# VITA-Group/Open-L2O

Measured on AMD Instinct MI355X. Metric: unroll-steps/sec (batch x params x T), L2O-DM on Quadratic d=128, higher is better.
Workload: dtype f32

## Files before the change

### open_l2o_amd/csrc/l2o_unroll.hip

```cpp
#include "l2o_host.h"
#include "l2o_step.h"
#include "l2o_problem_fg.h"
#include "l2o_unroll.h"
#include "l2o_unroll_pair.h"
#include "l2o_unroll_lds.h"
#include "l2o_unroll_cu.h"
#include "l2o_unroll_cu8.h"
#include "l2o_ilp_kernels.h"

__global__ void k_combine_halves(const float* __restrict__ fx_half, float* __restrict__ fx_part, int nb, int nparts,
                                 float inv_bg, float* __restrict__ fx, unsigned long long* __restrict__ xbuf, long xwords,
                                 PairWs* ws, int b0, int B_local);
__global__ void k_coresident_probe(unsigned* ctr, unsigned* min_seen);

static int check_problem(const l2o_problem* p) {
  if (!p) return fail(L2O_ERR_ARG, "problem is NULL");
  if (p->B_local <= 0 || p->B_global < p->B_local || p->D <= 0)
    return fail(L2O_ERR_ARG, "bad problem sizes B_local=%d B_global=%d D=%d", p->B_local, p->B_global, p->D);
  switch (p->kind) {
    case L2O_PROB_SIMPLE: return L2O_OK;
    case L2O_PROB_QUADRATIC:
    case L2O_PROB_LASSO:
      if (!p->W || !p->y || p->M <= 0) return fail(L2O_ERR_ARG, "problem needs W, y and M > 0");
      if (p->kind == L2O_PROB_QUADRATIC && p->M != p->D) return fail(L2O_ERR_ARG, "quadratic needs M == D");
      return L2O_OK;
    case L2O_PROB_RASTRIGIN:
    case L2O_PROB_SQUARE_COS:
      if (!p->W || !p->y || !p->C || p->M != p->D)
        return fail(L2O_ERR_ARG, "rastrigin / square_cos need W, y, C and M == D");
      return L2O_OK;
    default: return fail(L2O_ERR_UNSUPPORTED, "problem kind %d has no HIP kernel", p->kind);
  }
}

struct UnrollGeom { int CH, nw; size_t lds; };
static bool unroll_geom(const l2o_problem* p, UnrollGeom* g) {
  const int D = p->D, M = p->M;
  g->nw = tiles_per_problem(D);
  if (g->nw > 8 || M > 16 * g->nw) return false;
  const int need = g->nw;
  g->CH = need <= 1 ? 1 : (need <= 2 ? 2 : (need <= 4 ? 4 : 8));
  const int SQ = 16 * g->CH, S = SQ + 16;
  g->lds = sizeof(float) * (2 * (size_t)SQ * S + 3 * (size_t)SQ + 8);
  return g->lds <= 160 * 1024;
}

static int pair_chunk(const l2o_problem* p, const UnrollGeom& g, hipStream_t s) {
  if (!opt(L2O_OPT_PAIR) || g.CH < 2) return 0;
  const int cap = coresident_cus(s) / 2;
  if (p->B_local <= cap) return p->B_local;
  if (cap < 8) return 0;
  const int n = (p->B_local + cap - 1) / cap;
  const int chunk = (((p->B_local + n - 1) / n) + 7) & ~7;
  return chunk <= cap ? chunk : (cap & ~7);
}
struct PairLayout { size_t xbuf_off, xbuf_bytes, fxh_off, total; int npg; size_t lds; };
static PairLayout pair_layout(const l2o_problem* p, const UnrollGeom& g, int T) {
  PairLayout L;
  const int SQ = 16 * g.CH;
  L.npg = SQ;
  L.xbuf_off = sizeof(PairWs);
  L.xbuf_bytes = (size_t)p->B_local * 2 * 2 * L.npg * sizeof(unsigned long long);
  L.fxh_off = L.xbuf_off + L.xbuf_bytes;
  L.total = L.fxh_off + sizeof(float) * (size_t)(T + 1) * g.CH * p->B_local;
  L.lds = 0;
  return L;
}

template <int PRE, int KIND>
static int launch_unroll_ch(const UnrollArgs& a, const UnrollGeom& g, hipStream_t s, const l2o_problem* prob,
                            void* workspace, float* fx, bool* fx_done) {
  const bool hist = a.hist_st != nullptr;
  int chunk = workspace ? pair_chunk(prob, g, s) : 0;
  {
    const int one_lds = (int)opt(L2O_OPT_ONE_LDS);
#ifdef L2O_LDS_ABL_ANYNW
    const bool shape_ok = g.nw >= 1 && a.pp.M <= 16 * g.nw;
#else
    const bool shape_ok = g.CH == 8 && g.nw >= 5;
#endif
    const bool plain = !(opt(L2O_OPT_EXACT_GATES) && !hist);
    if ((one_lds == 2 || (one_lds == 1 && (chunk == 0 || a.pp.B_local > chunk))) && shape_ok && plain) {
      UnrollArgs al = a;
      al.ticks = workspace ? &reinterpret_cast<PairWs*>(workspace)->ticks : nullptr;
      void (*fl)(UnrollArgs) = hist ? k_unroll_lds<PRE, KIND, true> : k_unroll_lds<PRE, KIND, false>;
      const size_t lds = sizeof(float) * ((size_t)LstmCoreLds<PRE>::kFragWords + 2 * 128 + 8);
      const int rc = launch(fl, dim3(a.pp.B_local), dim3(64 * g.nw), lds, s, al);
      if (rc) return rc;
      note_form(L2O_FORM_UNROLL_LDS);
      note_variant(0, hist, false, false, 0, 0);
      return L2O_OK;
    }
  }
  if (chunk > 0) {
    const PairLayout L = pair_layout(prob, g, a.T);
    UnrollPairArgs pa;
    pa.u = a;
    pa.ws = reinterpret_cast<PairWs*>(workspace);
    pa.xbuf = reinterpret_cast<unsigned long long*>(static_cast<char*>(workspace) + L.xbuf_off);
    pa.fx_half = reinterpret_cast<float*>(static_cast<char*>(workspace) + L.fxh_off);
    pa.use_salt = a.T + 1 < 0xffff ? 1u : 0u;
    pa.plain_stores = opt(L2O_OPT_PAIR_PLAIN_STORES) ? 1u : 0u;
    pa.b0 = 0;
    pa.nb = a.pp.B_local;
    const int B = a.pp.B_local;
    const bool one_launch = chunk >= B;
    const bool exact = opt(L2O_OPT_EXACT_GATES) != 0 && !hist;
    bool fast_launched = false;
    {
      void (*fn)(UnrollPairArgs) = nullptr;
      const size_t dyn_lds = L.lds;
      const int SQ = 16 * g.CH;
      const bool fast = opt(L2O_OPT_PAIR_FAST_LOAD) != 0 && a.pp.M == SQ && a.pp.D == SQ;
      pa.fast_load = fast ? 1u : 0u;
      fast_launched = fast;
#define L2O_PAIR_FN(C)                                                                                       \
  (fast ? (hist ? k_unroll_pair<PRE, KIND, C, true, false, true>                                             \
                : (exact ? k_unroll_pair<PRE, KIND, C, false, true, true> : k_unroll_pair<PRE, KIND, C, false, false, true>)) \
        : (hist ? k_unroll_pair<PRE, KIND, C, true> : (exact ? k_unroll_pair<PRE, KIND, C, false, true> : k_unroll_pair<PRE, KIND, C, false>)))
      switch (g.CH) {
        case 2: fn = L2O_PAIR_FN(2); break;
        case 4: fn = L2O_PAIR_FN(4); break;
        default: fn = L2O_PAIR_FN(8); break;
      }
#undef L2O_PAIR_FN
      for (int b0 = 0; b0 < B; b0 += chunk) {
        pa.b0 = b0;
        pa.nb = B - b0 < chunk ? B - b0 : chunk;
        hipLaunchKernelGGL(fn, dim3((pa.nb + 7) / 8 * 16), dim3(64 * (g.CH / 2)), dyn_lds, s, pa);
        HIP_TRY(hipGetLastError());
        hipLaunchKernelGGL(k_combine_halves, dim3(a.T + 1), dim3(256), 0, s, pa.fx_half, a.fx_part, pa.nb, g.CH,
                           a.pp.inv_bg, one_launch ? fx : nullptr, pa.xbuf, (long)pa.nb * 2 * 2 * L.npg, pa.ws, b0, B);
        HIP_TRY(hipGetLastError());
      }
    }
    note_form(L2O_FORM_UNROLL_PAIR, (B + chunk - 1) / chunk);
    note_variant(g.CH, hist, exact, fast_launched, 0, 0);
    if (fx_done) *fx_done = fx != nullptr && one_launch;
    return L2O_OK;
  }
  void (*fn)(UnrollArgs) = nullptr;
  const bool exact1 = opt(L2O_OPT_EXACT_GATES) != 0 && !hist;
  switch (g.CH) {
    case 1: fn = hist ? k_unroll<PRE, KIND, 1, true> : (exact1 ? k_unroll<PRE, KIND, 1, false, true> : k_unroll<PRE, KIND, 1, false>); break;
    case 2: fn = hist ? k_unroll<PRE, KIND, 2, true> : (exact1 ? k_unroll<PRE, KIND, 2, false, true> : k_unroll<PRE, KIND, 2, false>); break;
    case 4: fn = hist ? k_unroll<PRE, KIND, 4, true> : (exact1 ? k_unroll<PRE, KIND, 4, false, true> : k_unroll<PRE, KIND, 4, false>); break;
    default: fn = hist ? k_unroll<PRE, KIND, 8, true> : k_unroll<PRE, KIND, 8, false>; break;
  }
  const int rc = launch(fn, dim3(a.pp.B_local), dim3(64 * g.nw), g.lds, s, a);
  if (rc) return rc;
  note_form(L2O_FORM_UNROLL);
  note_variant(g.CH, hist, exact1 && g.CH <= 4, false, 0, 0);
  return L2O_OK;
}

template <int PRE>
static int launch_unroll_kind(const UnrollArgs& a, const UnrollGeom& g, int kind, hipStream_t s,
                              const l2o_problem* prob, void* workspace, float* fx, bool* fx_done) {
  switch (kind) {
    case L2O_PROB_QUADRATIC: return launch_unroll_ch<PRE, L2O_PROB_QUADRATIC>(a, g, s, prob, workspace, fx, fx_done);
    case L2O_PROB_LASSO: return launch_unroll_ch<PRE, L2O_PROB_LASSO>(a, g, s, prob, workspace, fx, fx_done);
    case L2O_PROB_RASTRIGIN: return launch_unroll_ch<PRE, L2O_PROB_RASTRIGIN>(a, g, s, prob, workspace, fx, fx_done);
    case L2O_PROB_SQUARE_COS: return launch_unroll_ch<PRE, L2O_PROB_SQUARE_COS>(a, g, s, prob, workspace, fx, fx_done);
    default: return fail(L2O_ERR_UNSUPPORTED, "no fused kernel for problem kind %d", kind);
  }
}

static bool unroll_cu_eligible(const l2o_problem* p) {
  if (!opt(L2O_OPT_UNROLL_CU)) return false;
  if (p->D < 4 || p->D > 512 || (p->D & 3) || p->M <= 0) return false;
  return unroll_cu_layout(p->D).lds + sizeof(float) * bx::kBiasWords <= 160 * 1024;
}
template <int PRE, int KR>
static int launch_unroll_cu8(const UnrollArgs& a, hipStream_t s) {
  const UnrollCu8Layout L = unroll_cu8_layout(a.pp.D, PRE, KR);
  const bool hist = a.hist_st != nullptr;
  void (*fn)(UnrollArgs) = a.pp.D <= 256 ? (hist ? k_unroll_cu8<PRE, 1, KR, true> : k_unroll_cu8<PRE, 1, KR, false>)
                                         : (hist ? k_unroll_cu8<PRE, 2, KR, true> : k_unroll_cu8<PRE, 2, KR, false>);
  note_form(L2O_FORM_UNROLL_CU8);
  note_variant(0, hist, false, false, KR, a.pp.D <= 256 ? 1 : 2);
  return launch(fn, dim3(a.pp.B_local), dim3(kCu8Threads), L.lds, s, a);
}
template <int PRE>
static int launch_unroll_cu(const UnrollArgs& a_in, hipStream_t s) {
  const int form = (int)opt(L2O_OPT_UNROLL_CU);
  const bool hist0 = a_in.hist_st != nullptr;
  auto fits = [&](int kr) { return unroll_cu8_layout(a_in.pp.D, PRE, kr).lds + sizeof(float) * bx::kBiasWords <= 160 * 1024; };
  int KR = 0;
  if (form == 1) {
    KR = hist0 ? 2 : (PRE == L2O_PRE_FC_ELU ? 4 : 3);
    if (hist0 && !fits(2) && PRE != L2O_PRE_FC_ELU) KR = 3;
  } else if (form >= 3 && form <= 5) KR = 7 - form;
  if (KR && fits(KR))
    return KR == 4 ? launch_unroll_cu8<PRE, 4>(a_in, s) : (KR == 3 ? launch_unroll_cu8<PRE, 3>(a_in, s) : launch_unroll_cu8<PRE, 2>(a_in, s));
  const UnrollCuLayout L = unroll_cu_layout(a_in.pp.D);
  const UnrollArgs& a = a_in;
  const bool hist = a.hist_st != nullptr;
  void (*fn)(UnrollArgs) = a.pp.D <= 256 ? (hist ? k_unroll_cu<PRE, 1, true> : k_unroll_cu<PRE, 1, false>)
                                         : (hist ? k_unroll_cu<PRE, 2, true> : k_unroll_cu<PRE, 2, false>);
  note_form(L2O_FORM_UNROLL_CU);
  note_variant(0, hist, false, false, 0, a.pp.D <= 256 ? 1 : 2);
  return launch(fn, dim3(a.pp.B_local), dim3(kCuThreads), L.lds, s, a);
}

extern "C" {

static int launch_problem_fg(const ProbParams& pp, const float* x, float* f_part, float* g, void* stream) {
  const size_t lds = sizeof(float) * ((size_t)((pp.D + 3) & ~3) + ((pp.M + 3) & ~3) + 4 * kFgThreads + kFgWaves);
  if (lds > 160 * 1024) return fail(L2O_ERR_UNSUPPORTED, "problem too large for k_problem_fg (D=%d M=%d)", pp.D, pp.M);
  const bool vec = pp.kind != L2O_PROB_SIMPLE && (pp.D & 3) == 0 && ((uintptr_t)pp.W & 15) == 0;
  if (vec && pp.D >= 64 && pp.D <= 2048 && ((uintptr_t)x & 15) == 0 && (!pp.x_scale || ((uintptr_t)pp.x_scale & 15) == 0) &&
      !pp.w_shared && !opt(L2O_OPT_FG_TWO_PASS)) {
    const size_t lds1 = sizeof(float) * ((size_t)kFgWaves * pp.D + kFgWaves);
    void (*f1)(ProbParams, const float*, float*, float*) =
        pp.D <= 256 ? k_problem_fg1<1> : pp.D <= 512 ? k_problem_fg1<2> : pp.D <= 1024 ? k_problem_fg1<4> : k_problem_fg1<8>;
// ... 250 lines not shown
```

### open_l2o_amd/csrc/l2o_unroll_pair.h

```cpp
#pragma once
#include "l2o_lstm_bx3.h"
#include "l2o_params.h"

struct PairWs {
  unsigned status;
  unsigned seq;
  unsigned fault;
  unsigned pad0;
  long long ticks;
  long long ticks_total;
  unsigned pad[8];
  long long phases[16];
};
static_assert(sizeof(PairWs) == 64 + 128, "workspace header layout (include/l2o_abi.h)");

struct UnrollPairArgs {
  UnrollArgs u;
  PairWs* ws;
  unsigned long long* xbuf;
  float* fx_half;
  unsigned use_salt;
  unsigned plain_stores;
  int b0, nb;
  unsigned fast_load;
};

__device__ __forceinline__ unsigned long long pack_granule(float v, unsigned tag) {
  return ((unsigned long long)tag << 32) | (unsigned long long)__float_as_uint(v);
}

template <int N>
__device__ __forceinline__ void lds_read_f4(float4 (&v)[N], const float* p) {
  const unsigned addr = (unsigned)(size_t)(__attribute__((address_space(3))) const char*)p;
  static_assert(N == 1 || N == 2 || N == 4 || N == 8, "");
  if constexpr (N == 1)
    asm volatile("ds_read_b128 %0, %1\n\ts_waitcnt lgkmcnt(0)" : "=&v"(v[0]) : "v"(addr) : "memory");
  if constexpr (N == 2)
    asm volatile("ds_read_b128 %0, %2\n\tds_read_b128 %1, %2 offset:64\n\ts_waitcnt lgkmcnt(0)"
                 : "=&v"(v[0]), "=&v"(v[1]) : "v"(addr) : "memory");
  if constexpr (N == 4)
    asm volatile("ds_read_b128 %0, %4\n\tds_read_b128 %1, %4 offset:64\n\tds_read_b128 %2, %4 offset:128\n\t"
                 "ds_read_b128 %3, %4 offset:192\n\ts_waitcnt lgkmcnt(0)"
                 : "=&v"(v[0]), "=&v"(v[1]), "=&v"(v[2]), "=&v"(v[3]) : "v"(addr) : "memory");
  if constexpr (N == 8)
    asm volatile("ds_read_b128 %0, %8\n\tds_read_b128 %1, %8 offset:64\n\tds_read_b128 %2, %8 offset:128\n\t"
                 "ds_read_b128 %3, %8 offset:192\n\tds_read_b128 %4, %8 offset:256\n\tds_read_b128 %5, %8 offset:320\n\t"
                 "ds_read_b128 %6, %8 offset:384\n\tds_read_b128 %7, %8 offset:448\n\ts_waitcnt lgkmcnt(0)"
                 : "=&v"(v[0]), "=&v"(v[1]), "=&v"(v[2]), "=&v"(v[3]), "=&v"(v[4]), "=&v"(v[5]), "=&v"(v[6]), "=&v"(v[7])
                 : "v"(addr) : "memory");
}

template <int N>
__device__ __forceinline__ void lds_load_f4(l2o::f32x4 (&v)[N], const float* p) {
  const auto* q = reinterpret_cast<const __attribute__((address_space(3))) l2o::f32x4*>(
      (const __attribute__((address_space(3))) float*)p);
#pragma unroll
  for (int m = 0; m < N; ++m) v[m] = q[4 * m];
}
__device__ __forceinline__ void dot4v(const float4 a, const l2o::f32x4 b, float4& acc) {
  acc.x = __builtin_fmaf(a.x, b[0], acc.x);
  acc.y = __builtin_fmaf(a.y, b[1], acc.y);
  acc.z = __builtin_fmaf(a.z, b[2], acc.z);
  acc.w = __builtin_fmaf(a.w, b[3], acc.w);
}

#ifndef L2O_GEMV_PK
#define L2O_GEMV_PK 1
#endif
#ifndef L2O_GEMV_PK_G
#define L2O_GEMV_PK_G L2O_GEMV_PK
#endif
struct Acc4pk { l2o::bx::f32x2 lo, hi; };
__device__ __forceinline__ void dot4pk(const l2o::f32x4 a, const l2o::f32x4 b, Acc4pk& acc) {
  acc.lo = __builtin_elementwise_fma(__builtin_shufflevector(a, a, 0, 1), __builtin_shufflevector(b, b, 0, 1), acc.lo);
  acc.hi = __builtin_elementwise_fma(__builtin_shufflevector(a, a, 2, 3), __builtin_shufflevector(b, b, 2, 3), acc.hi);
}
__device__ __forceinline__ float hsum4pk(const Acc4pk& a) { return (a.lo.x + a.lo.y) + (a.hi.x + a.hi.y); }
__device__ __forceinline__ l2o::f32x4 as_quad(const float4 v) { return l2o::f32x4{v.x, v.y, v.z, v.w}; }
__device__ __forceinline__ void dot4q(const l2o::f32x4 a, const l2o::f32x4 b, float4& acc) {
  acc.x = __builtin_fmaf(a[0], b[0], acc.x);
  acc.y = __builtin_fmaf(a[1], b[1], acc.y);
  acc.z = __builtin_fmaf(a[2], b[2], acc.z);
  acc.w = __builtin_fmaf(a[3], b[3], acc.w);
}

#ifndef L2O_PAIR_LDS_BARRIERS
#define L2O_PAIR_LDS_BARRIERS 0
#endif
#ifdef L2O_PROFILE_PHASES
#define L2O_LAUNCH_MARK(i)                                                                  \
  do {                                                                                      \
    __builtin_amdgcn_sched_barrier(0);                                                      \
    launch_marks[i] = (unsigned)(__builtin_readcyclecounter() - kernel_t0);                 \
    __builtin_amdgcn_sched_barrier(0);                                                      \
  } while (0)
#define L2O_LAUNCH_MARK_LANDED(i)                                                           \
  do {                                                                                      \
    __builtin_amdgcn_sched_barrier(0);                                                      \
    asm volatile("s_waitcnt vmcnt(0) lgkmcnt(0)" ::: "memory");                             \
    L2O_LAUNCH_MARK(i);                                                                     \
  } while (0)
#else
#define L2O_LAUNCH_MARK(i) do {} while (0)
#define L2O_LAUNCH_MARK_LANDED(i) do {} while (0)
#endif

template <int PRE, int KIND, int CH, bool HIST, bool EXACT>
__device__ __forceinline__ void unroll_pair_body_gather(const UnrollPairArgs& pa) {
  const long long kernel_t0 = __builtin_readcyclecounter();
#ifdef L2O_PROFILE_PHASES
  unsigned launch_marks[8] = {0, 0, 0, 0, 0, 0, 0, 0};
#endif
  constexpr int SQ = 16 * CH;
  constexpr int NWH = CH / 2;
  constexpr int NC = 16 * NWH;
  __shared__ __attribute__((aligned(16))) float xs[NC];
  __shared__ __attribute__((aligned(16))) float rs[SQ];
  const UnrollArgs& a = pa.u;
  const ProbParams& pp = a.pp;
  const int D = pp.D, M = pp.M;
  const int tid = threadIdx.x, lane = tid & 63, wv = tid >> 6;
  const int c = lane & 15, q = lane >> 4;
  const int bid = blockIdx.x;
  const unsigned salt = pa.use_salt ? ((pa.ws->seq + 1u) & 0x7fffu) << 16 : 0u;
#ifdef L2O_PROFILE_PHASES
  asm volatile("" ::"s"(salt));
#endif
  L2O_LAUNCH_MARK(0);
  const int half = (bid >> 3) & 1;
  const int bl = ((bid >> 4) << 3) | (bid & 7);
  if (bl >= pa.nb) return;
  const int b = pa.b0 + bl;
  const int tile_in_prob = half * NWH + wv;
  const int gq = q, gr = c;

  const float* Wb = pp.W + (pp.w_shared ? (size_t)0 : (size_t)b * M * D);
  const int col0 = half * NC;
  float4 wr[2][NWH], wt[CH];
#pragma unroll
  for (int p = 0; p < 2; ++p) {
    const int row = (2 * wv + p) * kTile + gr;
#pragma unroll
    for (int m = 0; m < NWH; ++m) {
      float e[4];
#pragma unroll
      for (int k = 0; k < 4; ++k) {
        const int col = col0 + 16 * m + 4 * gq + k;
        e[k] = (row < M && col < D) ? Wb[(size_t)row * D + col] : 0.0f;
      }
      wr[p][m] = make_float4(e[0], e[1], e[2], e[3]);
    }
  }
  {
    const int col = col0 + wv * kTile + gr;
#pragma unroll
    for (int m = 0; m < CH; ++m) {
      float e[4];
#pragma unroll
      for (int k = 0; k < 4; ++k) {
        const int row = 16 * m + 4 * gq + k;
        e[k] = (row < M && col < D) ? Wb[(size_t)row * D + col] : 0.0f;
      }
      wt[m] = make_float4(e[0], e[1], e[2], e[3]);
    }
  }
  constexpr bool kPk = L2O_GEMV_PK != 0;
  l2o::f32x4 wrq[2][NWH], wtq[CH];
#pragma unroll
  for (int m = 0; m < NWH; ++m) { wrq[0][m] = as_quad(wr[0][m]); wrq[1][m] = as_quad(wr[1][m]); }
#pragma unroll
  for (int m = 0; m < CH; ++m) wtq[m] = as_quad(wt[m]);
  const int myrow = (2 * wv + (gq & 1)) * kTile + gr;
  const float myy = (gq < 2 && myrow < M) ? pp.y[(size_t)b * M + myrow] : 0.0f;
  const bool row_counted = gq < 2 && (half == 0 ? (myrow < NC) : (myrow >= NC));

  using Core = LstmCorePair<PRE, !EXACT, false>;
  Core core;
  core.load(a.np.wpack, lane);
  core.pin();
  __shared__ __attribute__((aligned(16))) float bias_s[Core::kBiasFloats];
  core.stage_bias(bias_s, a.np.wpack, tid, blockDim.x, q);
  L2O_LAUNCH_MARK(1);
  const int j = tile_in_prob * kTile + c;
  const bool live = j < D;
  const size_t idx = (size_t)b * D + j;
  const int tpp = (D + kTile - 1) / kTile;
  const bool tile_real = tile_in_prob < tpp;
  TileState s;
  float* st_tile = a.st + ((size_t)b * tpp + (tile_real ? tile_in_prob : 0)) * kStateFloatsPerTile;
  if (tile_real && !a.zero_state) load_tile_state(s, st_tile, lane);
  else {
#pragma unroll
    for (int t = 0; t < kNT; ++t) s.h1[t] = s.c1[t] = s.h2[t] = s.c2[t] = 0.0f;
  }
  float xv = live ? (a.x_in ? a.x_in : a.x)[idx] : 0.0f;
  const float sc = (live && pp.x_scale) ? pp.x_scale[idx] : 1.0f;
  float cj = 0.0f;
  constexpr bool kCos = KIND == L2O_PROB_RASTRIGIN || KIND == L2O_PROB_SQUARE_COS;
  if (kCos) cj = live ? pp.C[idx] : 0.0f;
  float mv = 0.0f, vv = 0.0f;
  if (PRE == L2O_PRE_FC_ELU && !a.zero_state) { mv = live ? a.m[idx] : 0.0f; vv = live ? a.v[idx] : 0.0f; }
  float p1h = a.p1_hi, p1l = a.p1_lo, p2h = a.p2_hi, p2l = a.p2_lo;
  constexpr bool kSq = KIND == L2O_PROB_QUADRATIC || KIND == L2O_PROB_SQUARE_COS;
  const float coef = kSq ? 1.0f : 0.5f;
  const float cg = (KIND == L2O_PROB_QUADRATIC ? 2.0f : 1.0f) * pp.inv_bg;
  const float kTwoPi = pp.twopi;
  const float* xsq = xs + 4 * gq;
  const float* rsq = rs + 4 * gq;
  unsigned long long* mine = pa.xbuf + ((size_t)bl * 2 + half) * 2 * SQ;
  const unsigned long long* theirs = pa.xbuf + ((size_t)bl * 2 + (half ^ 1)) * 2 * SQ;
  bool dead = false;
  if (pa.ws->fault != 0) {
    dead = true;
    if (tid == 0) atomicExch(&pa.ws->status, 1u);
  }
  L2O_LAUNCH_MARK_LANDED(2);
  __shared__ __attribute__((aligned(16))) int same_xcd_s4[4];
  int& same_xcd_s = same_xcd_s4[0];
  if (tid == 0) {
    unsigned my_xcc;
    asm volatile("s_getreg_b32 %0, hwreg(HW_REG_XCC_ID)" : "=s"(my_xcc));
    my_xcc &= 0xfu;
    const unsigned kHsTag = 0x80000000u | salt | 0xffffu;
    __hip_atomic_store(mine + SQ, ((unsigned long long)kHsTag << 32) | my_xcc, __ATOMIC_RELAXED, __HIP_MEMORY_SCOPE_AGENT);
    unsigned long long g = 0;
    int spins = 0;
    bool ok = true;
#pragma nounroll
    for (;;) {
      g = __hip_atomic_load(theirs + SQ, __ATOMIC_RELAXED, __HIP_MEMORY_SCOPE_AGENT);
      if ((unsigned)(g >> 32) == kHsTag) break;
      if (dead || ++spins > (1 << 20)) { ok = false; break; }
      __builtin_amdgcn_s_sleep(1);
    }
    same_xcd_s = ok && pa.plain_stores && ((unsigned)g & 0xfu) == my_xcc;
  }
  __syncthreads();
  const bool same_xcd = same_xcd_s != 0;
  L2O_LAUNCH_MARK(3);

  constexpr bool kBiasRegs = kPairBiasRegs<PRE, KIND, CH, HIST, EXACT, false>;
#define L2O_PAIR_FX_PTR 0
#include "l2o_unroll_pair_loop.h"
#undef L2O_PAIR_FX_PTR
}

template <int PRE, int KIND, int CH, bool HIST, bool EXACT>
__device__ __forceinline__ void unroll_pair_body(const UnrollPairArgs& pa) {
  const long long kernel_t0 = __builtin_readcyclecounter();
#ifdef L2O_PROFILE_PHASES
  unsigned launch_marks[8] = {0, 0, 0, 0, 0, 0, 0, 0};
#endif
  constexpr int SQ = 16 * CH;
  constexpr int NWH = CH / 2;
  constexpr int NC = 16 * NWH;
  __shared__ __attribute__((aligned(16))) float xs[NC];
  __shared__ __attribute__((aligned(16))) float rs[SQ];
  const UnrollArgs& a = pa.u;
  const ProbParams& pp = a.pp;
  const int D = pp.D, M = pp.M;
  const int tid = threadIdx.x, lane = tid & 63, wv = tid >> 6;
  const int c = lane & 15, q = lane >> 4;
  const int bid = blockIdx.x;
  const int half = (bid >> 3) & 1;
  const int bl = ((bid >> 4) << 3) | (bid & 7);
  if (bl >= pa.nb) return;
  const int b = pa.b0 + bl;
  const int tile_in_prob = half * NWH + wv;
  const int gq = q, gr = c;

  using Core = LstmCorePair<PRE, !EXACT, true>;
  constexpr bool kStage = Core::kStageFrags > 0 && NWH >= 2;
  __shared__ float4 frag_stage[kStage ? Core::kStageFrags * 64 : 1];
  static_assert(sizeof(frag_stage) + sizeof(float) * (NC + SQ + Core::kBiasFloats + 4) <= 64 * 1024, "static LDS");
  if constexpr (kStage) {
    const int wvs = __builtin_amdgcn_readfirstlane(wv);
    const float* src = a.np.wpack + Core::kStageOff + lane * 4;
#pragma unroll
    for (int f = 0; f < (Core::kStageFrags + NWH - 1) / NWH; ++f) {
      const int fr = NWH * f + wvs;
      if (Core::kStageFrags % NWH == 0 || fr < Core::kStageFrags)
        __builtin_amdgcn_global_load_lds((gbl_void*)(src + fr * bx::kFragWords), (lds_void*)(frag_stage + fr * 64), 16, 0, 0);
    }
  }

  const float* Wb = pp.W + (pp.w_shared ? (size_t)0 : (size_t)b * M * D);
  const int col0 = half * NC;
  float4 wr[2][NWH], wt[CH];
  if (pa.fast_load && M == SQ && D == SQ && (reinterpret_cast<size_t>(pp.W) & 15) == 0) {
    const float4* Wq = reinterpret_cast<const float4*>(Wb + (size_t)(2 * wv * kTile + gr) * SQ + col0 + 4 * gq);
#pragma unroll
    for (int p = 0; p < 2; ++p)
#pragma unroll
      for (int m = 0; m < NWH; ++m) wr[p][m] = Wq[(p * kTile * SQ + 16 * m) / 4];
    const float* Wc = Wb + (size_t)(4 * gq) * SQ + col0 + wv * kTile + gr;
#pragma unroll
    for (int m = 0; m < CH; ++m)
      wt[m] = make_float4(Wc[(16 * m + 0) * SQ], Wc[(16 * m + 1) * SQ], Wc[(16 * m + 2) * SQ], Wc[(16 * m + 3) * SQ]);
  } else {
#pragma unroll
    for (int p = 0; p < 2; ++p) {
      const int row = (2 * wv + p) * kTile + gr;
#pragma unroll
      for (int m = 0; m < NWH; ++m) {
        float e[4];
#pragma unroll
        for (int k = 0; k < 4; ++k) {
          const int col = col0 + 16 * m + 4 * gq + k;
          e[k] = (row < M && col < D) ? Wb[(size_t)row * D + col] : 0.0f;
        }
        wr[p][m] = make_float4(e[0], e[1], e[2], e[3]);
      }
    }
    const int col = col0 + wv * kTile + gr;
#pragma unroll
    for (int m = 0; m < CH; ++m) {
      float e[4];
#pragma unroll
      for (int k = 0; k < 4; ++k) {
        const int row = 16 * m + 4 * gq + k;
        e[k] = (row < M && col < D) ? Wb[(size_t)row * D + col] : 0.0f;
      }
      wt[m] = make_float4(e[0], e[1], e[2], e[3]);
    }
  }
  unsigned hdr_lane = 0;
  asm volatile("" : "+v"(hdr_lane));
  const unsigned* hdr = &pa.ws->seq + hdr_lane;
  const unsigned seq_v = hdr[0], fault_v = hdr[1];
  static_assert(offsetof(PairWs, fault) == offsetof(PairWs, seq) + sizeof(unsigned), "seq and fault are neighbours");
  const int myrow = (2 * wv + (gq & 1)) * kTile + gr;
  const float y_ld = pp.y[(size_t)b * M + (myrow < M ? myrow : 0)];
  const bool row_counted = gq < 2 && (half == 0 ? (myrow < NC) : (myrow >= NC));
// ... 25 lines not shown
    core.load(a.np.wpack, lane);
  __builtin_amdgcn_sched_barrier(0);
  L2O_LAUNCH_MARK(1);

  if constexpr (kStage) {
    L2O_LAUNCH_MARK_LANDED(2);
    asm volatile("s_waitcnt vmcnt(0)" ::: "memory");
  }
  const unsigned seq_w = __builtin_amdgcn_readfirstlane(seq_v), fault_w = __builtin_amdgcn_readfirstlane(fault_v);
  const unsigned salt = pa.use_salt ? ((seq_w + 1u) & 0x7fffu) << 16 : 0u;
  unsigned long long* mine = pa.xbuf + ((size_t)bl * 2 + half) * 2 * SQ;
  const unsigned long long* theirs = pa.xbuf + ((size_t)bl * 2 + (half ^ 1)) * 2 * SQ;
  const unsigned kHsTag = 0x80000000u | salt | 0xffffu;
  unsigned my_xcc = 0;
  if (tid == 0) {
    asm volatile("s_getreg_b32 %0, hwreg(HW_REG_XCC_ID)" : "=s"(my_xcc));
    my_xcc &= 0xfu;
    __hip_atomic_store(mine + SQ, ((unsigned long long)kHsTag << 32) | my_xcc, __ATOMIC_RELAXED, __HIP_MEMORY_SCOPE_AGENT);
  }
  L2O_LAUNCH_MARK(0);
  __builtin_amdgcn_sched_barrier(0);
  __shared__ __attribute__((aligned(16))) float bias_s[Core::kBiasFloats];
  if constexpr (kStage) core.template put_bias<64 * NWH>(bias_s, bias_ld, tid, q);
  else core.stage_bias(bias_s, a.np.wpack, tid, 64 * NWH, q);
  if constexpr (kStage) {
    asm volatile("s_waitcnt lgkmcnt(0)" ::: "memory");
    __builtin_amdgcn_s_barrier();
    asm volatile("" ::: "memory");
    core.read_stage(frag_stage, lane);
    __builtin_amdgcn_sched_barrier(0);
  } else
    core.pin();
  constexpr bool kPk = L2O_GEMV_PK != 0;
  l2o::f32x4 wrq[2][NWH], wtq[CH];
#pragma unroll
  for (int m = 0; m < NWH; ++m) { wrq[0][m] = as_quad(wr[0][m]); wrq[1][m] = as_quad(wr[1][m]); }
#pragma unroll
  for (int m = 0; m < CH; ++m) wtq[m] = as_quad(wt[m]);
  TileState s;
  unpack_tile_state(s, st_ld);
  if (!(tile_real && !a.zero_state)) {
#pragma unroll
    for (int t = 0; t < kNT; ++t) s.h1[t] = s.c1[t] = s.h2[t] = s.c2[t] = 0.0f;
  }
  const float myy = (gq < 2 && myrow < M) ? y_ld : 0.0f;
  float xv = live ? x_ld : 0.0f;
  const float sc = live ? sc_ld : 1.0f;
  const float cj = live ? cj_ld : 0.0f;
  float mv = live ? m_ld : 0.0f, vv = live ? v_ld : 0.0f;
  float p1h = a.p1_hi, p1l = a.p1_lo, p2h = a.p2_hi, p2l = a.p2_lo;
  constexpr bool kSq = KIND == L2O_PROB_QUADRATIC || KIND == L2O_PROB_SQUARE_COS;
  const float coef = kSq ? 1.0f : 0.5f;
  const float cg = (KIND == L2O_PROB_QUADRATIC ? 2.0f : 1.0f) * pp.inv_bg;
  const float kTwoPi = pp.twopi;
  const float* xsq = xs + 4 * gq;
  const float* rsq = rs + 4 * gq;
  bool dead = false;
  if (fault_w != 0) {
    dead = true;
    if (tid == 0) atomicExch(&pa.ws->status, 1u);
  }
  if constexpr (!kStage) L2O_LAUNCH_MARK_LANDED(2);
  __shared__ __attribute__((aligned(16))) int same_xcd_s4[4];
  int& same_xcd_s = same_xcd_s4[0];
  if (tid == 0) {
    unsigned long long g = 0;
    int spins = 0;
    bool ok = true;
#pragma nounroll
    for (;;) {
      g = __hip_atomic_load(theirs + SQ, __ATOMIC_RELAXED, __HIP_MEMORY_SCOPE_AGENT);
      if ((unsigned)(g >> 32) == kHsTag) break;
      if (dead || ++spins > (1 << 20)) { ok = false; break; }
      __builtin_amdgcn_s_sleep(1);
    }
    same_xcd_s = ok && pa.plain_stores && ((unsigned)g & 0xfu) == my_xcc;
  }
  __syncthreads();
  const bool same_xcd = same_xcd_s != 0;
  if constexpr (kStage) core.pin();
  L2O_LAUNCH_MARK(3);

  constexpr bool kBiasRegs = kPairBiasRegs<PRE, KIND, CH, HIST, EXACT, true>;
#define L2O_PAIR_FX_PTR 1
#include "l2o_unroll_pair_loop.h"
#undef L2O_PAIR_FX_PTR
}

template <int PRE, int KIND, int CH, bool HIST, bool EXACT = false, bool FAST = false>
__global__ __launch_bounds__(256) void k_unroll_pair(UnrollPairArgs pa) {
  if constexpr (FAST) unroll_pair_body<PRE, KIND, CH, HIST, EXACT>(pa);
  else unroll_pair_body_gather<PRE, KIND, CH, HIST, EXACT>(pa);
}
```

### open_l2o_amd/csrc/l2o_unroll_pair_loop.h

```cpp
  f32x4 acc1[kNT], acc2[kNT];
  core.init(s, q);
  if constexpr (kBiasRegs) {
    core.hold_bias();
    core.arm(acc1, acc2);
  } else
    core.preload(acc1, acc2);
  PhaseClock pc;
  pc.start();

  xs[wv * kTile + c] = live ? xv * sc : 0.0f;
  const size_t hist_n = (size_t)pp.B_local * D;
  const bool pub_plain = gq < 2 && same_xcd;
  unsigned poll_salt = salt | (dead ? 0x80000000u : 0u);
#ifdef L2O_ABLATE_EXCHANGE
  poll_salt = salt | 0x80000000u;
#endif
#if L2O_PAIR_FX_PTR
  float* fxp = pa.fx_half + (size_t)bl * (2 * NWH) + half * NWH + wv;
  const size_t fx_stride = (size_t)pa.nb * (2 * NWH);
#endif
  L2O_LAUNCH_MARK(4);
  const long long loop_t0 = __builtin_readcyclecounter();
  if constexpr (!HIST) {
    for (int t = 0; t < a.T; ++t) {
#include "l2o_unroll_pair_step_head.h"
#include "l2o_unroll_pair_step_tail.h"
    }
    {
      const int t = a.T;
#include "l2o_unroll_pair_step_head.h"
    }
  } else
  for (int t = 0;; ++t) {
#include "l2o_unroll_pair_step_head.h"
    if (t == a.T && !HIST) break;
#include "l2o_unroll_pair_step_tail.h"
  }
  L2O_LAUNCH_MARK(5);
#ifdef L2O_PROFILE_PHASES
  if (blockIdx.x == 0 && tid == 0) pc.dump(pa.ws->phases);
#endif
  if (bid == 0 && tid == 0) pa.ws->ticks = __builtin_readcyclecounter() - loop_t0;

  if (live && q == 0) {
    a.x[idx] = xv;
    if (PRE == L2O_PRE_FC_ELU) { a.m[idx] = mv; a.v[idx] = vv; }
  }
  if (tile_real) store_tile_state(s, st_tile, lane);
  if (bid == 0 && tid == 0) pa.ws->ticks_total = __builtin_readcyclecounter() - kernel_t0;
  L2O_LAUNCH_MARK(6);
  L2O_LAUNCH_MARK_LANDED(7);
#ifdef L2O_PROFILE_PHASES
  if (bid == 0 && tid == 0) {
#pragma unroll
    for (int i = 0; i < 8; ++i) pa.ws->pad[i] = launch_marks[i];
  }
#endif
```

### open_l2o_amd/csrc/l2o_unroll_pair_step_head.h

```cpp
    const float xsv = xv * sc;
    const unsigned tag = salt | ((unsigned)t + 1u);
    const int par = t & 1;
    pc.mark(0);
    if (HIST || L2O_PAIR_LDS_BARRIERS) lds_barrier(); else __syncthreads();
    pc.mark(2);
    float part;
    {
      float4 r0 = {0.f, 0.f, 0.f, 0.f}, r1 = {0.f, 0.f, 0.f, 0.f};
      Acc4pk r0p = {{0.f, 0.f}, {0.f, 0.f}}, r1p = {{0.f, 0.f}, {0.f, 0.f}};
      l2o::f32x4 x4v[NWH];
      lds_load_f4<NWH>(x4v, xsq);
      core.refresh(s);
      __builtin_amdgcn_sched_group_barrier(0x100, NWH, 0);
      __builtin_amdgcn_sched_group_barrier(0x002, 48, 0);
#pragma unroll
      for (int m = 0; m < NWH; ++m) {
        if (kPk) { dot4pk(wrq[0][m], x4v[m], r0p); dot4pk(wrq[1][m], x4v[m], r1p); }
        else { dot4v(wr[0][m], x4v[m], r0); dot4v(wr[1][m], x4v[m], r1); }
      }
      const float h0 = kPk ? hsum4pk(r0p) : hsum4(r0), h1 = kPk ? hsum4pk(r1p) : hsum4(r1);
      const u32x2 sw = __builtin_amdgcn_permlane16_swap(__float_as_uint(h0), __float_as_uint(h1), false, false);
      part = xor32_add(__uint_as_float(sw[0]) + __uint_as_float(sw[1]));
    }
    {
      unsigned long long* const pub = mine + par * SQ + myrow;
      if (__builtin_expect(!same_xcd, 0)) {
        asm volatile("");
        if (gq < 2) __hip_atomic_store(pub, pack_granule(part, tag), __ATOMIC_RELAXED, __HIP_MEMORY_SCOPE_AGENT);
      }
      if (pub_plain) __hip_atomic_store(pub, pack_granule(part, tag), __ATOMIC_RELAXED, __HIP_MEMORY_SCOPE_WORKGROUP);
    }
    l2o::SinCos trig = {0.0f, 1.0f};
    if (kCos) trig = l2o::sincos_f(kTwoPi * xsv);
    pc.mark(3);
#ifndef L2O_PAIR_POLL_AT
#define L2O_PAIR_POLL_AT 20
#endif
    constexpr int kPollAt = L2O_PAIR_POLL_AT < Core::kTotal ? L2O_PAIR_POLL_AT : Core::kTotal;
    constexpr int kPollAt1 = L2O_PAIR_POLL_AT > Core::kTotal ? L2O_PAIR_POLL_AT - Core::kTotal : 0;
    core.template issue_l2_prev<0, kPollAt>(s, acc2);
    if (kPollAt1 > 0) core.template issue_l1_prev<0, kPollAt1>(s, acc1);
    const unsigned long long* src = theirs + par * SQ + (gq < 2 ? myrow : 0);
    unsigned long long g = 0;
    const unsigned poll_tag = poll_salt | ((unsigned)t + 1u);
    __builtin_amdgcn_sched_barrier(0);
#ifndef L2O_ABLATE_EXCHANGE
    if (gq < 2) g = __hip_atomic_load(src, __ATOMIC_RELAXED, __HIP_MEMORY_SCOPE_AGENT);
#endif
    __builtin_amdgcn_sched_barrier(0);
    if (kPollAt < Core::kTotal) core.template issue_l2_prev<kPollAt, Core::kTotal>(s, acc2);
    core.template issue_l1_prev<kPollAt1, Core::kTotal>(s, acc1);
    float contrib = 0.0f;
    if (gq < 2) {
      int spins = 0;
#ifdef L2O_ABLATE_EXCHANGE
      const bool wait = false;
#else
      const bool wait = (unsigned)(g >> 32) != poll_tag;
#endif
      if (__builtin_expect(__builtin_amdgcn_ballot_w64(wait) != 0, 0)) {
        asm volatile("");
        bool timed_out = false;
        if (poll_salt != salt) g = 0;
        else if (wait) {
#pragma nounroll
          for (;;) {
            g = __hip_atomic_load(src, __ATOMIC_RELAXED, __HIP_MEMORY_SCOPE_AGENT);
            if ((unsigned)(g >> 32) == tag) break;
            if (++spins > (1 << 20)) { timed_out = true; atomicExch(&pa.ws->status, 1u); break; }
#ifndef L2O_POLL_NOSLEEP
            __builtin_amdgcn_s_sleep(1);
#endif
          }
        }
        if (__builtin_amdgcn_ballot_w64(timed_out) != 0) poll_salt = salt | 0x80000000u;
      }
      const float r = (part + __uint_as_float((unsigned)g)) - myy;
      rs[myrow] = r;
      if (row_counted) contrib = coef * r * r;
    }
    if (live && q == 0) {
      if (KIND == L2O_PROB_LASSO) contrib += pp.l1 * __builtin_fabsf(xsv);
      if (kCos) contrib += pp.alpha - pp.alpha * cj * trig.c;
    }
    if (HIST && t < a.T && tile_real)
// ... 19 lines not shown
```

### open_l2o_amd/csrc/l2o_unroll_pair_step_tail.h

```cpp
    constexpr bool kPkG = L2O_GEMV_PK_G != 0;
    float4 gacc4 = {0.f, 0.f, 0.f, 0.f};
    Acc4pk gaccp = {{0.f, 0.f}, {0.f, 0.f}};
#pragma unroll
    for (int m = 0; m < CH; ++m) {
      if (kPkG) dot4pk(wtq[m], rv4v[m], gaccp);
      else dot4v(wt[m], rv4v[m], gacc4);
    }
    float gv = quad_q_sum(kPkG ? hsum4pk(gaccp) : hsum4(gacc4));
    if (KIND == L2O_PROB_SQUARE_COS) gv *= 2.0f;
    if (KIND == L2O_PROB_LASSO) gv += pp.l1 * (xsv > 0.f ? 1.f : (xsv < 0.f ? -1.f : 0.f));
    if (kCos) gv += kTwoPi * pp.alpha * cj * trig.s;
    gv = live ? gv * cg * sc : 0.0f;
    if (HIST && live && q == 0) {
      if (t < a.T) a.hist_g[(size_t)t * hist_n + idx] = gv;
      else a.hist_gfinal[idx] = gv;
    }
    if (HIST && t == a.T) break;

    float in0, in1;
    if (PRE == L2O_PRE_FC_ELU) {
      rnnprop_inputs(gv, mv, vv, a.np.beta1, a.np.beta2, a.np.omb1, a.np.omb2, 1.0f - p1h, 1.0f - p2h, in0, in1);
      if (HIST && live && q == 0) { a.hist_m[(size_t)t * hist_n + idx] = mv; a.hist_v[(size_t)t * hist_n + idx] = vv; }
      if (!live) { in0 = 0.0f; in1 = 0.0f; }
      {
        float hi = p1h * a.np.beta1, er = __builtin_fmaf(p1h, a.np.beta1, -hi);
        float lo = __builtin_fmaf(p1l, a.np.beta1, er), sum = hi + lo;
        p1l = lo - (sum - hi); p1h = sum;
        hi = p2h * a.np.beta2; er = __builtin_fmaf(p2h, a.np.beta2, -hi);
        lo = __builtin_fmaf(p2l, a.np.beta2, er); sum = hi + lo;
        p2l = lo - (sum - hi); p2h = sum;
      }
    } else {
      preprocess_grad<PRE>(gv, a.np.k_inv_ln2, a.np.exp_k, in0, in1);
    }
    float d = core.template finish<false, bx::NoShadow, false>(s, acc1, acc2, in0, in1, q, pc);
    if (__builtin_expect(a.np.tanh_output != 0, 0)) {
      asm volatile("");
      d = tanhf_(d);
    }
    xv = __builtin_fmaf(d, a.np.scale, xv);
    __builtin_amdgcn_sched_barrier(0);
    xs[wv * kTile + c] = live ? xv * sc : 0.0f;
    __builtin_amdgcn_sched_barrier(0);
    if constexpr (kBiasRegs) core.arm(acc1, acc2);
    else core.preload_unpinned(acc1, acc2);
    __builtin_amdgcn_sched_barrier(0);
    pc.mark(9);
```

### open_l2o_amd/csrc/l2o_util_kernels.h

```cpp
#pragma once
#include "l2o_bwd_mfma.h"
#include "l2o_unroll_pair.h"

__global__ void k_state_repack(float* __restrict__ h1, float* __restrict__ c1, float* __restrict__ h2,
                               float* __restrict__ c2, float* __restrict__ st, int B, int D, int tpp,
                               int to_packed) {
  const size_t gid = (size_t)blockIdx.x * blockDim.x + threadIdx.x;
  const size_t total = (size_t)B * tpp * 64 * 20;
  if (gid >= total) return;
  const int e = gid % 20;
  const int lane = (gid / 20) % 64;
  const size_t tile = gid / (20 * 64);
  const int b = tile / tpp, tw = tile % tpp;
  const int c = lane & 15, q = lane >> 4;
  const int j = tw * kTile + c;
  const int arr = e / 5, t = e % 5, u = 4 * t + q;
  const size_t paddr = tile * kStateFloatsPerTile + ((size_t)(e >> 2) * 64 + lane) * 4 + (e & 3);
  float* ref = arr == 0 ? h1 : (arr == 1 ? c1 : (arr == 2 ? h2 : c2));
  if (j < D) {
    const size_t raddr = ((size_t)b * D + j) * kH + u;
    if (to_packed) st[paddr] = ref[raddr];
    else ref[raddr] = st[paddr];
  } else if (to_packed) {
    st[paddr] = 0.0f;
  }
}

__global__ void k_reduce_fx(const float* __restrict__ fx_part, int T1, int B_local, float inv_bg,
                            float* __restrict__ fx) {
  const int t = blockIdx.x;
  const int lane = threadIdx.x;
  float acc = 0.0f;
  for (int b = lane; b < B_local; b += 64) acc += fx_part[(size_t)t * B_local + b];
  acc = wave_sum64(acc);
  if (lane == 0) fx[t] = acc * inv_bg;
}

__global__ __launch_bounds__(256) void k_combine_halves(const float* __restrict__ fx_half, float* __restrict__ fx_part,
                                                        int nb, int nparts, float inv_bg, float* __restrict__ fx,
                                                        unsigned long long* __restrict__ xbuf, long xwords, PairWs* ws,
                                                        int b0, int B_local) {
  const int t = blockIdx.x, tid = threadIdx.x, lane = tid & 63;
  if (tid >= 64) {
    const long npairs = xwords >> 1;
    const long per2 = (npairs + gridDim.x - 1) / gridDim.x;
    const long lo = (long)t * per2, hi = lo + per2 < npairs ? lo + per2 : npairs;
    ulonglong2* xpair = reinterpret_cast<ulonglong2*>(xbuf);
    for (long e = lo + (tid - 64); e < hi; e += 192) xpair[e] = make_ulonglong2(0ull, 0ull);
    return;
  }
  const bool bump = t == 0 && tid == 0;
  unsigned seq0 = 0;
  if (bump) seq0 = ws->seq;
  float acc = 0.0f;
  if (nb <= 128 && (nparts == 2 || nparts == 4 || nparts == 8)) {
    const int bA = lane, bB = lane + 64;
    const bool hA = bA < nb, hB = bB < nb;
    const float* pA = fx_half + ((size_t)t * nb + (hA ? bA : 0)) * nparts;
    const float* pB = fx_half + ((size_t)t * nb + (hB ? bB : 0)) * nparts;
    float fA, fB;
    if (nparts == 8) {
      const float4 a0 = *reinterpret_cast<const float4*>(pA), a1 = *reinterpret_cast<const float4*>(pA + 4);
      const float4 c0 = *reinterpret_cast<const float4*>(pB), c1 = *reinterpret_cast<const float4*>(pB + 4);
      fA = ((a0.x + a0.y) + a0.z) + a0.w;
      fA = (((fA + a1.x) + a1.y) + a1.z) + a1.w;
      fB = ((c0.x + c0.y) + c0.z) + c0.w;
      fB = (((fB + c1.x) + c1.y) + c1.z) + c1.w;
    } else if (nparts == 4) {
      const float4 a0 = *reinterpret_cast<const float4*>(pA), c0 = *reinterpret_cast<const float4*>(pB);
      fA = ((a0.x + a0.y) + a0.z) + a0.w;
      fB = ((c0.x + c0.y) + c0.z) + c0.w;
    } else {
      const float2 a0 = *reinterpret_cast<const float2*>(pA), c0 = *reinterpret_cast<const float2*>(pB);
      fA = a0.x + a0.y;
      fB = c0.x + c0.y;
    }
    if (hA) { fx_part[(size_t)t * B_local + b0 + bA] = fA; acc += fA; }
    if (hB) { fx_part[(size_t)t * B_local + b0 + bB] = fB; acc += fB; }
  } else {
    for (int b = lane; b < nb; b += 64) {
      const float* p = fx_half + ((size_t)t * nb + b) * nparts;
      float f = p[0];
      for (int k = 1; k < nparts; ++k) f += p[k];
      fx_part[(size_t)t * B_local + b0 + b] = f;
      acc += f;
    }
  }
  if (fx) {
    acc = l2o::wave_sum64(acc);
    if (lane == 0) fx[t] = acc * inv_bg;
  }
  if (bump) {
    if (xwords & 1) xbuf[xwords - 1] = 0ull;
    ws->seq = seq0 + 1u;
  }
}

__global__ __launch_bounds__(256) void k_coresident_probe(unsigned* ctr, unsigned* min_seen) {
  extern __shared__ float probe_lds[];
  if (threadIdx.x == 0) {
    probe_lds[0] = 1.0f;
    atomicAdd(ctr, 1u);
    for (int i = 0; i < 8; ++i) __builtin_amdgcn_s_sleep(127);
    const unsigned v = __hip_atomic_load(ctr, __ATOMIC_RELAXED, __HIP_MEMORY_SCOPE_AGENT);
    atomicMin(min_seen, v);
  }
}

extern "C" {
__host__ __device__ static inline uint16_t bf16_rne(float f) {
  uint32_t u = __builtin_bit_cast(uint32_t, f);
  u += 0x7fffu + ((u >> 16) & 1u);
  return (uint16_t)(u >> 16);
}
__host__ __device__ static inline double bf16_value(uint16_t h) {
  return (double)__builtin_bit_cast(float, (uint32_t)h << 16);
}
__host__ __device__ static inline void bf16_split3(double v, uint16_t (&out)[3]) {
  for (int s = 0; s < 3; ++s) {
    out[s] = bf16_rne((float)v);
    v -= bf16_value(out[s]);
  }
}

// ... 148 lines not shown
```

Before: 10.75 billion.

## Unroll pair time loop by two with constant parity and add boundary profiling

Manually unrolls the pair kernel's time-step loop by two, so the double-buffer parity is a compile-time constant in each half. This removes parity-dependent indexing and may let the compiler schedule across adjacent steps. In the unrolled path, the two-sum momentum update is rewritten to use FMAs. Separately, adds kernel-boundary timestamp recording to the workspace under the profiling build flag. The unroll raises code size and register pressure, and the FMA-based compensated sum may change rounding slightly.

```diff
diff --git a/open_l2o_amd/csrc/l2o_unroll.hip b/open_l2o_amd/csrc/l2o_unroll.hip
--- a/open_l2o_amd/csrc/l2o_unroll.hip
+++ b/open_l2o_amd/csrc/l2o_unroll.hip
@@ -10,7 +10,11 @@
 
 __global__ void k_combine_halves(const float* __restrict__ fx_half, float* __restrict__ fx_part, int nb, int nparts,
                                  float inv_bg, float* __restrict__ fx, unsigned long long* __restrict__ xbuf, long xwords,
-                                 PairWs* ws, int b0, int B_local);
+                                 PairWs* ws, int b0, int B_local
+#ifdef L2O_PROFILE_PHASES
+                                 , unsigned long long* dbg
+#endif
+                                 );
 __global__ void k_coresident_probe(unsigned* ctr, unsigned* min_seen);
 
 static int check_problem(const l2o_problem* p) {
@@ -54,7 +58,7 @@
   const int chunk = (((p->B_local + n - 1) / n) + 7) & ~7;
   return chunk <= cap ? chunk : (cap & ~7);
 }
-struct PairLayout { size_t xbuf_off, xbuf_bytes, fxh_off, total; int npg; size_t lds; };
+struct PairLayout { size_t xbuf_off, xbuf_bytes, fxh_off, total; int npg; size_t lds; size_t dbg_off = 0; };
 static PairLayout pair_layout(const l2o_problem* p, const UnrollGeom& g, int T) {
   PairLayout L;
   const int SQ = 16 * g.CH;
@@ -64,6 +68,10 @@
   L.fxh_off = L.xbuf_off + L.xbuf_bytes;
   L.total = L.fxh_off + sizeof(float) * (size_t)(T + 1) * g.CH * p->B_local;
   L.lds = 0;
+#ifdef L2O_PROFILE_PHASES
+  L.dbg_off = (L.total + 15) & ~(size_t)15;
+  L.total = L.dbg_off + sizeof(unsigned long long) * kBoundaryWords;
+#endif
   return L;
 }
 
@@ -103,6 +111,9 @@
     pa.plain_stores = opt(L2O_OPT_PAIR_PLAIN_STORES) ? 1u : 0u;
     pa.b0 = 0;
     pa.nb = a.pp.B_local;
+#ifdef L2O_PROFILE_PHASES
+    pa.dbg = reinterpret_cast<unsigned long long*>(static_cast<char*>(workspace) + L.dbg_off);
+#endif
     const int B = a.pp.B_local;
     const bool one_launch = chunk >= B;
     const bool exact = opt(L2O_OPT_EXACT_GATES) != 0 && !hist;
@@ -130,7 +141,11 @@
         hipLaunchKernelGGL(fn, dim3((pa.nb + 7) / 8 * 16), dim3(64 * (g.CH / 2)), dyn_lds, s, pa);
         HIP_TRY(hipGetLastError());
         hipLaunchKernelGGL(k_combine_halves, dim3(a.T + 1), dim3(256), 0, s, pa.fx_half, a.fx_part, pa.nb, g.CH,
-                           a.pp.inv_bg, one_launch ? fx : nullptr, pa.xbuf, (long)pa.nb * 2 * 2 * L.npg, pa.ws, b0, B);
+                           a.pp.inv_bg, one_launch ? fx : nullptr, pa.xbuf, (long)pa.nb * 2 * 2 * L.npg, pa.ws, b0, B
+#ifdef L2O_PROFILE_PHASES
+                           , pa.dbg
+#endif
+                           );
         HIP_TRY(hipGetLastError());
       }
     }
diff --git a/open_l2o_amd/csrc/l2o_unroll_pair.h b/open_l2o_amd/csrc/l2o_unroll_pair.h
--- a/open_l2o_amd/csrc/l2o_unroll_pair.h
+++ b/open_l2o_amd/csrc/l2o_unroll_pair.h
@@ -23,7 +23,18 @@
   unsigned plain_stores;
   int b0, nb;
   unsigned fast_load;
+#ifdef L2O_PROFILE_PHASES
+  unsigned long long* dbg;
+#endif
 };
+
+#ifdef L2O_PROFILE_PHASES
+constexpr int kBoundaryRing = 8, kBoundaryWgs = 1024;
+constexpr size_t kBoundaryWords = 8 + (size_t)kBoundaryRing * 2 * kBoundaryWgs * 2;
+__device__ __forceinline__ unsigned long long* boundary_slot(unsigned long long* dbg, unsigned ring, int kernel, int wg) {
+  return dbg + 8 + (((size_t)ring * 2 + kernel) * kBoundaryWgs + wg) * 2;
+}
+#endif
 
 __device__ __forceinline__ unsigned long long pack_granule(float v, unsigned tag) {
   return ((unsigned long long)tag << 32) | (unsigned long long)__float_as_uint(v);
@@ -106,9 +117,14 @@
 #endif
 
 template <int PRE, int KIND, int CH, bool HIST, bool EXACT>
+constexpr bool kPairUnroll2 =
+    !HIST && !EXACT && !(PRE == L2O_PRE_LOGSIGN && (KIND == L2O_PROB_RASTRIGIN || KIND == L2O_PROB_SQUARE_COS) && CH == 8);
+
+template <int PRE, int KIND, int CH, bool HIST, bool EXACT>
 __device__ __forceinline__ void unroll_pair_body_gather(const UnrollPairArgs& pa) {
   const long long kernel_t0 = __builtin_readcyclecounter();
 #ifdef L2O_PROFILE_PHASES
+  const unsigned long long boundary_in = __builtin_amdgcn_s_memrealtime();
   unsigned launch_marks[8] = {0, 0, 0, 0, 0, 0, 0, 0};
 #endif
   constexpr int SQ = 16 * CH;
@@ -241,7 +257,9 @@
 
   constexpr bool kBiasRegs = kPairBiasRegs<PRE, KIND, CH, HIST, EXACT, false>;
 #define L2O_PAIR_FX_PTR 0
+#define L2O_PAIR_UNROLL2 0
 #include "l2o_unroll_pair_loop.h"
+#undef L2O_PAIR_UNROLL2
 #undef L2O_PAIR_FX_PTR
 }
 
@@ -249,6 +267,7 @@
 __device__ __forceinline__ void unroll_pair_body(const UnrollPairArgs& pa) {
   const long long kernel_t0 = __builtin_readcyclecounter();
 #ifdef L2O_PROFILE_PHASES
+  const unsigned long long boundary_in = __builtin_amdgcn_s_memrealtime();
   unsigned launch_marks[8] = {0, 0, 0, 0, 0, 0, 0, 0};
 #endif
   constexpr int SQ = 16 * CH;
@@ -440,8 +459,11 @@
   L2O_LAUNCH_MARK(3);
 
   constexpr bool kBiasRegs = kPairBiasRegs<PRE, KIND, CH, HIST, EXACT, true>;
+  constexpr bool kUnroll2 = kPairUnroll2<PRE, KIND, CH, HIST, EXACT>;
 #define L2O_PAIR_FX_PTR 1
+#define L2O_PAIR_UNROLL2 1
 #include "l2o_unroll_pair_loop.h"
+#undef L2O_PAIR_UNROLL2
 #undef L2O_PAIR_FX_PTR
 }
 
diff --git a/open_l2o_amd/csrc/l2o_unroll_pair_loop.h b/open_l2o_amd/csrc/l2o_unroll_pair_loop.h
--- a/open_l2o_amd/csrc/l2o_unroll_pair_loop.h
+++ b/open_l2o_amd/csrc/l2o_unroll_pair_loop.h
@@ -21,6 +21,35 @@
 #endif
   L2O_LAUNCH_MARK(4);
   const long long loop_t0 = __builtin_readcyclecounter();
+#if L2O_PAIR_UNROLL2
+  if constexpr (!HIST && kUnroll2) {
+    int t = 0;
+    for (; t + 1 < a.T; ++t) {
+      {
+#define L2O_PAIR_PAR 0
+#include "l2o_unroll_pair_step_head.h"
+#include "l2o_unroll_pair_step_tail.h"
+#undef L2O_PAIR_PAR
+      }
+      ++t;
+      {
+#define L2O_PAIR_PAR 1
+#include "l2o_unroll_pair_step_head.h"
+#include "l2o_unroll_pair_step_tail.h"
+#undef L2O_PAIR_PAR
+      }
+    }
+    for (; t < a.T; ++t) {
+#define L2O_PAIR_PAR 0
+#include "l2o_unroll_pair_step_head.h"
+#include "l2o_unroll_pair_step_tail.h"
+#undef L2O_PAIR_PAR
+    }
+    {
+#include "l2o_unroll_pair_step_head.h"
+    }
+  } else
+#endif
   if constexpr (!HIST) {
     for (int t = 0; t < a.T; ++t) {
 #include "l2o_unroll_pair_step_head.h"
@@ -55,4 +84,12 @@
 #pragma unroll
     for (int i = 0; i < 8; ++i) pa.ws->pad[i] = launch_marks[i];
   }
+  __syncthreads();
+  if (tid == 0 && bid < kBoundaryWgs) {
+    const unsigned ring = pa.ws->seq & (kBoundaryRing - 1);
+    unsigned long long* d = boundary_slot(pa.dbg, ring, 0, bid);
+    d[0] = boundary_in;
+    d[1] = __builtin_amdgcn_s_memrealtime();
+    if (bid == 0) pa.dbg[0] = ring;
+  }
 #endif
diff --git a/open_l2o_amd/csrc/l2o_unroll_pair_step_head.h b/open_l2o_amd/csrc/l2o_unroll_pair_step_head.h
--- a/open_l2o_amd/csrc/l2o_unroll_pair_step_head.h
+++ b/open_l2o_amd/csrc/l2o_unroll_pair_step_head.h
@@ -1,6 +1,10 @@
     const float xsv = xv * sc;
     const unsigned tag = salt | ((unsigned)t + 1u);
+#ifdef L2O_PAIR_PAR
+    constexpr int par = L2O_PAIR_PAR;
+#else
     const int par = t & 1;
+#endif
     pc.mark(0);
     if (HIST || L2O_PAIR_LDS_BARRIERS) lds_barrier(); else __syncthreads();
     pc.mark(2);
diff --git a/open_l2o_amd/csrc/l2o_unroll_pair_step_tail.h b/open_l2o_amd/csrc/l2o_unroll_pair_step_tail.h
--- a/open_l2o_amd/csrc/l2o_unroll_pair_step_tail.h
+++ b/open_l2o_amd/csrc/l2o_unroll_pair_step_tail.h
@@ -24,11 +24,19 @@
       if (!live) { in0 = 0.0f; in1 = 0.0f; }
       {
         float hi = p1h * a.np.beta1, er = __builtin_fmaf(p1h, a.np.beta1, -hi);
+#ifdef L2O_PAIR_PAR
+        float lo = __builtin_fmaf(p1l, a.np.beta1, er), sum = __builtin_fmaf(a.np.beta1, p1h, lo);
+        p1l = lo - __builtin_fmaf(-a.np.beta1, p1h, sum); p1h = sum;
+        hi = p2h * a.np.beta2; er = __builtin_fmaf(p2h, a.np.beta2, -hi);
+        lo = __builtin_fmaf(p2l, a.np.beta2, er); sum = __builtin_fmaf(a.np.beta2, p2h, lo);
+        p2l = lo - __builtin_fmaf(-a.np.beta2, p2h, sum); p2h = sum;
+#else
         float lo = __builtin_fmaf(p1l, a.np.beta1, er), sum = hi + lo;
         p1l = lo - (sum - hi); p1h = sum;
         hi = p2h * a.np.beta2; er = __builtin_fmaf(p2h, a.np.beta2, -hi);
         lo = __builtin_fmaf(p2l, a.np.beta2, er); sum = hi + lo;
         p2l = lo - (sum - hi); p2h = sum;
+#endif
       }
     } else {
       preprocess_grad<PRE>(gv, a.np.k_inv_ln2, a.np.exp_k, in0, in1);
diff --git a/open_l2o_amd/csrc/l2o_util_kernels.h b/open_l2o_amd/csrc/l2o_util_kernels.h
--- a/open_l2o_amd/csrc/l2o_util_kernels.h
+++ b/open_l2o_amd/csrc/l2o_util_kernels.h
@@ -39,7 +39,22 @@
 __global__ __launch_bounds__(256) void k_combine_halves(const float* __restrict__ fx_half, float* __restrict__ fx_part,
                                                         int nb, int nparts, float inv_bg, float* __restrict__ fx,
                                                         unsigned long long* __restrict__ xbuf, long xwords, PairWs* ws,
-                                                        int b0, int B_local) {
+                                                        int b0, int B_local
+#ifdef L2O_PROFILE_PHASES
+                                                        , unsigned long long* dbg
+#endif
+                                                        ) {
+#ifdef L2O_PROFILE_PHASES
+  const unsigned long long boundary_in = __builtin_amdgcn_s_memrealtime();
+  struct BoundaryOut {
+    unsigned long long* d;
+    __device__ ~BoundaryOut() {
+      asm volatile("s_waitcnt vmcnt(0)" ::: "memory");
+      if ((threadIdx.x & 63) == 0 && d) atomicMax(d + 1, (unsigned long long)__builtin_amdgcn_s_memrealtime());
+    }
+  } boundary_out{blockIdx.x < kBoundaryWgs ? boundary_slot(dbg, (unsigned)dbg[0] & (kBoundaryRing - 1), 1, blockIdx.x) : nullptr};
+  if (threadIdx.x == 0 && boundary_out.d) boundary_out.d[0] = boundary_in;
+#endif
   const int t = blockIdx.x, tid = threadIdx.x, lane = tid & 63;
   if (tid >= 64) {
     const long npairs = xwords >> 1;
```

After: 10.86 billion, median of 6. About the same (+1.0%).
